# tachyon-beep/keisei

Hardware: AMD Instinct MI355X
Metric: PPO samples/sec, se_resnet 40x256 on 50x9x9 (higher is better)
Workload: dtype bf16; 1 GPU; se_resnet 40x256 KataGo-PPO minibatch step (gather+fwd+loss+bwd+clip+Adam), minibatch 4096/GPU from a 16384-sample device-resident epoch dataset, obs 50x9x9; per_gpu_batch=4096, global_batch=4096, parallelism=dp1

## Files before the change

keisei_amd/csrc/common.h:

```cpp
#pragma once
#include <hip/hip_runtime.h>
#include <stdint.h>

#define KA_OK 0
#define KA_ERR_ARG (-1)
#define KA_ERR_HIP (-2)
#define KA_ERR_UNSUPPORTED (-3)

#define KA_DTYPE_F32 0
#define KA_DTYPE_BF16 1

#define KA_BOARD 81
#define KA_PADBOARD 121

typedef __attribute__((ext_vector_type(8))) __bf16 bf16x8;
typedef __attribute__((ext_vector_type(4))) __bf16 bf16x4;
typedef __attribute__((ext_vector_type(4))) float f32x4;
typedef __attribute__((ext_vector_type(2))) float f32x2;

struct bf16_t { uint16_t v; };

void ka_set_error(const char* fmt, ...);
int ka_check_launch(const char* what);
#define KA_REQUIRE(cond, ...) do { if (!(cond)) { ka_set_error(__VA_ARGS__); return KA_ERR_ARG; } } while (0)

#include <atomic>
inline int ka_big_lds_once(const void* func, std::atomic<unsigned long long>& done, const char* what) {
    int dev = 0;
    if (hipGetDevice(&dev) != hipSuccess) { ka_set_error("%s: hipGetDevice failed", what); return KA_ERR_HIP; }
    const unsigned long long bit = 1ull << (dev & 63);
    if (done.load(std::memory_order_acquire) & bit) return KA_OK;
    if (hipFuncSetAttribute(func, hipFuncAttributeMaxDynamicSharedMemorySize, 160 * 1024) != hipSuccess) {
        ka_set_error("%s: hipFuncSetAttribute failed on device %d", what, dev);
        return KA_ERR_HIP;
    }
    done.fetch_or(bit, std::memory_order_release);
    return KA_OK;
}

#include <stdlib.h>
inline const char* ka_diag_env(const char* name) {
#ifdef KA_DIAG
    return getenv(name);
#else
    (void)name;
    return nullptr;
#endif
}

#define KA_OPTIONS(X)                                                                                                      \
    X(CONV_P) X(CONV_MT) X(CONV_PC2) X(CONV_PC2_SKIP) X(CONV_PC2_STAG) X(CONV_CORNER_IN) X(CONV_P_STAG) X(CONV_P_PRIO) X(CONV_P_WGS) X(CONV_P_NPW) X(CONV_WM) X(CONV_KC)       \
    X(CONV_NTW) X(CONV_STAGGER) X(CONV_PRIO) X(WGRAD_TN) X(WGRAD_WGS) X(WGRAD_STAG) X(WGRAD_LEAN) X(BOARD_PAIRS) X(TF_LDS_EPI) X(TF_K256) X(TF_BIG)    \
    X(TF_MAP2D) X(TF_ATTN_LDS) X(TF_ATTN_ONE) X(TAIL_FWD_KB) X(TAIL_GATE_P4)
enum KaOpt {
#define KA_OPT_ENUM(n) KA_OPT_##n,
    KA_OPTIONS(KA_OPT_ENUM)
#undef KA_OPT_ENUM
    KA_OPT_COUNT
};
struct KaOptVal { int set, val; };
const KaOptVal* ka_opts();
inline bool ka_opt_set(KaOpt o) { return ka_opts()[o].set != 0; }
inline int ka_opt(KaOpt o, int dflt) { const KaOptVal v = ka_opts()[o]; return v.set ? v.val : dflt; }

std::atomic<unsigned long long*>& ka_debug_stamps();

enum KaConvRoute {
    KA_RT_CONV,
    KA_RT_PC,
    KA_RT_PC2,
    KA_RT_PC2_CORNER_IN,
    KA_RT_PC2_CORNER_OUT,
    KA_RT_CORNER,
    KA_RT_WGRAD_LEAN,
    KA_RT_WGRAD_TILED,
    KA_RT_COUNT
};
void ka_conv_route(int r);

__device__ __forceinline__ float bf2f(uint16_t h) { return __uint_as_float(((uint32_t)h) << 16); }
__device__ __forceinline__ uint16_t f2bf(float f) {
    __bf16 b = (__bf16)f;
    return __builtin_bit_cast(uint16_t, b);
}

template <typename T> struct Elem;
template <> struct Elem<float> {
    static constexpr int kSize = 4;
    static constexpr int kPer16 = 4;
    static constexpr int kDtype = KA_DTYPE_F32;
    typedef f32x4 vec16;
    static __device__ __forceinline__ float ld(const float* p) { return *p; }
    static __device__ __forceinline__ void st(float* p, float v) { *p = v; }
    static __device__ __forceinline__ void unpack(const vec16& v, float* f) {
        f[0] = v[0]; f[1] = v[1]; f[2] = v[2]; f[3] = v[3];
    }
    static __device__ __forceinline__ vec16 pack(const float* f) { vec16 v = {f[0], f[1], f[2], f[3]}; return v; }
};
template <> struct Elem<bf16_t> {
    static constexpr int kSize = 2;
    static constexpr int kPer16 = 8;
    static constexpr int kDtype = KA_DTYPE_BF16;
    typedef bf16x8 vec16;
    static __device__ __forceinline__ float ld(const bf16_t* p) { return bf2f(p->v); }
    static __device__ __forceinline__ void st(bf16_t* p, float v) { p->v = f2bf(v); }
    static __device__ __forceinline__ void unpack(const vec16& v, float* f) {
#pragma unroll
        for (int i = 0; i < 8; ++i) f[i] = (float)v[i];
    }
    static __device__ __forceinline__ vec16 pack(const float* f) {
        vec16 v;
#pragma unroll
        for (int i = 0; i < 8; ++i) v[i] = (__bf16)f[i];
        return v;
    }
};

template <typename T> __device__ __forceinline__ f32x2 ld2(const T* p);
template <> __device__ __forceinline__ f32x2 ld2<float>(const float* p) { return *reinterpret_cast<const f32x2*>(p); }
template <> __device__ __forceinline__ f32x2 ld2<bf16_t>(const bf16_t* p) {
    uint32_t u = *reinterpret_cast<const uint32_t*>(p);
    f32x2 r = {__uint_as_float(u << 16), __uint_as_float(u & 0xffff0000u)};
    return r;
}
template <typename T> __device__ __forceinline__ void st2(T* p, f32x2 v);
template <> __device__ __forceinline__ void st2<float>(float* p, f32x2 v) { *reinterpret_cast<f32x2*>(p) = v; }
template <> __device__ __forceinline__ void st2<bf16_t>(bf16_t* p, f32x2 v) {
    uint32_t u = (uint32_t)f2bf(v[0]) | ((uint32_t)f2bf(v[1]) << 16);
// ... 85 lines not shown
```

keisei_amd/csrc/conv3x3.hip:

```cpp
#include <stdlib.h>
#include <utility>
#include "common.h"

static std::atomic<long long> g_conv_routes[KA_RT_COUNT];
void ka_conv_route(int r) { g_conv_routes[r].fetch_add(1, std::memory_order_relaxed); }

namespace {

constexpr int kNB = 2;
constexpr int kPW = 17;
constexpr int kBoardStride = 193;
constexpr int kLdsSquares = kBoardStride + 11 * kPW;
constexpr int kImgSquares1 = 10 * kPW + 11;
constexpr int kZeroSquares = 2 * (kPW + 1) + 1;
__device__ __forceinline__ int lds_square(int b, int p) { return b * kBoardStride + (p / 9 + 1) * kPW + (p % 9) + 1; }
constexpr int kMTW = 6;

__host__ __device__ __forceinline__ int chan_of(int nt, int s, int NT) {
    return ((nt | 1) < NT) ? (nt >> 1) * 32 + (s >> 2) * 8 + (nt & 1) * 4 + (s & 3) : nt * 16 + s;
}

__device__ __forceinline__ float row_sum16(float v) {
    v += __int_as_float(__builtin_amdgcn_update_dpp(0, __float_as_int(v), 0xB1, 0xF, 0xF, true));
    v += __int_as_float(__builtin_amdgcn_update_dpp(0, __float_as_int(v), 0x4E, 0xF, 0xF, true));
// ... 765 lines not shown
                        const float d = (in && y * esc[e] + esh[e] > 0.f) ? (float)db : 0.f;
                        t1[e] += d; t2[e] += d * ((y - emu[e]) * eis[e]);
                        o[e] = (__bf16)d;
                    }
                    if (j == 0) o0[mt] = o;
                    else if (in) {
                        bf16x8 o8;
#pragma unroll
                        for (int e = 0; e < 4; ++e) { o8[e] = o0[mt][e]; o8[4 + e] = o[e]; }
                        *reinterpret_cast<bf16x8*>(static_cast<char*>(a.out) + ((size_t)(bb * KA_BOARD + p) * a.Cout + cb0) * 2) = o8;
                    }
                }
#pragma unroll
                for (int e = 0; e < 4; ++e) { t1[e] = row_sum16(t1[e]); t2[e] = row_sum16(t2[e]); }
                if (rl == 0) {
                    *reinterpret_cast<f32x4*>(a.ep_s1 + (size_t)bb * a.Cout + cb0 + 4 * j) = f32x4{t1[0], t1[1], t1[2], t1[3]};
                    *reinterpret_cast<f32x4*>(a.ep_s2 + (size_t)bb * a.Cout + cb0 + 4 * j) = f32x4{t2[0], t2[1], t2[2], t2[3]};
                }
            }
            wfrag(0, 0, w0); wfrag(0, 1, w1); wfrag(0, 2, w2);
        }
    }
}

template <bool TWO, bool MASKED, int NPW, int MT, bool STAG = false>
static int launch_conv_pc_form(const ConvArgs& a, int grid, size_t lds, hipStream_t st, const char* what) {
    static std::atomic<unsigned long long> done{0};
    if (int rc = ka_big_lds_once(reinterpret_cast<const void*>(&conv3x3_pc_kernel<TWO, MASKED, NPW, MT, STAG>), done, what)) return rc;
    hipLaunchKernelGGL((conv3x3_pc_kernel<TWO, MASKED, NPW, MT, STAG>), dim3(grid), dim3(512 + 64 * NPW), lds, st, a);
    return ka_check_launch(what);
}
static int launch_conv_pc(ConvArgs a, hipStream_t st) {
    a.tune_stagger = 0; a.tune_prio = 0;
    if (const char* e = ka_diag_env("KA_CONV_P_ABL")) a.tune_stagger = atoi(e);
    a.tune_prio = ka_opt(KA_OPT_CONV_P_PRIO, 0);
    ka_conv_route(KA_RT_PC);
    int grid = 256;
    if (const int v = ka_opt(KA_OPT_CONV_P_WGS, 0); v > 0) grid = v;
    if (grid > a.B) grid = a.B;
    const int stag = ka_opt(KA_OPT_CONV_P_STAG, 0);
#define KA_PC_FORM(TWO_, MASKED_, NPW_, LDS_, WHAT_)                                                         \
    (a.mt5 ? ((stag && !MASKED_) ? launch_conv_pc_form<TWO_, false, NPW_, 5, true>(a, grid, LDS_, st, WHAT_ ", 5 row tiles, staggered") \
                                 : launch_conv_pc_form<TWO_, MASKED_, NPW_, 5>(a, grid, LDS_, st, WHAT_ ", 5 row tiles"))            \
           : launch_conv_pc_form<TWO_, MASKED_, NPW_, kMTW>(a, grid, LDS_, st, WHAT_))
    if (a.in2 && a.ep_y) return KA_PC_FORM(true, true, 4, kPcLdsMasked, "conv3x3 (pc, masked)");
    if (a.in2) return KA_PC_FORM(true, false, 4, kPcLds, "conv3x3 (pc, two-tensor)");
    if (ka_opt_set(KA_OPT_CONV_P_NPW) ? ka_opt(KA_OPT_CONV_P_NPW, 4) == 2 : (a.in_scale || a.relu || a.in_bias))
        return KA_PC_FORM(false, false, 2, kPcLds, "conv3x3 (pc, 2 staging waves)");
    return KA_PC_FORM(false, false, 4, kPcLds, "conv3x3 (pc)");
#undef KA_PC_FORM
}

typedef __attribute__((ext_vector_type(2))) unsigned u32x2;
template <int C, int MT>
__device__ __forceinline__ void conv_epilogue_masked_pair(const ConvArgs& a, f32x4 (&acc)[2 * MT][2], int b0, bool has_b1, int nt0, int r, int q) {
    constexpr int ROWB = C * 2, NT = C / 16;
    const int cb[2] = {chan_of(nt0, 4 * q, NT), chan_of(nt0 + 1, 4 * q, NT)};
    const char* yb = static_cast<const char*>(a.ep_y) + (size_t)b0 * (KA_BOARD * ROWB);
    char* ob = static_cast<char*>(a.out) + (size_t)b0 * (KA_BOARD * ROWB);
    const int lo[2] = {r * ROWB + cb[0] * 2, r * ROWB + cb[1] * 2};
    auto live = [&](int mt) { return MT == 5 || mt < 5 || r == 0; };
    u32x2 yA[MT], yB[MT];
    auto yload = [&](int b, int j, u32x2 (&y)[MT]) {
#pragma unroll
        for (int mt = 0; mt < MT; ++mt) y[mt] = live(mt) ? *reinterpret_cast<const u32x2*>(yb + b * (KA_BOARD * ROWB) + lo[j] + mt * 16 * ROWB) : u32x2{0u, 0u};
    };
    f32x4 cA[2], cB[2];
    yload(0, 0, yA);
    cA[0] = *reinterpret_cast<const f32x4*>(a.ep_scale + cb[0]); cA[1] = *reinterpret_cast<const f32x4*>(a.ep_shift + cb[0]);
    if (a.bsum) {
#pragma unroll
        for (int b = 0; b < 2; ++b)
#pragma unroll
            for (int j = 0; j < 2; ++j) {
                float s0[4] = {0.f, 0.f, 0.f, 0.f};
#pragma unroll
                for (int mt = 0; mt < MT; ++mt)
#pragma unroll
                    for (int i = 0; i < 4; ++i) s0[i] += live(mt) ? acc[MT * b + mt][j][i] : 0.f;
#pragma unroll
                for (int i = 0; i < 4; ++i) s0[i] = row_sum16(s0[i]);
                if (r == 0 && (b == 0 || has_b1)) *reinterpret_cast<f32x4*>(a.bsum + (b0 + b) * C + cb[j]) = f32x4{s0[0], s0[1], s0[2], s0[3]};
            }
    }
    yload(0, 1, yB);
    cB[0] = *reinterpret_cast<const f32x4*>(a.ep_scale + cb[1]); cB[1] = *reinterpret_cast<const f32x4*>(a.ep_shift + cb[1]);
    auto process = [&](int b, int j, const u32x2 (&y)[MT], const f32x4 (&c)[2]) {
        const f32x4 emu = *reinterpret_cast<const f32x4*>(a.ep_mean + cb[j]), eis = *reinterpret_cast<const f32x4*>(a.ep_invstd + cb[j]);
        float t1[4] = {0.f, 0.f, 0.f, 0.f}, t2[4] = {0.f, 0.f, 0.f, 0.f};
#pragma unroll
        for (int mt = 0; mt < MT; ++mt) {
            u32x2 o;
#pragma unroll
            for (int h = 0; h < 2; ++h) {
                const unsigned yw = y[mt][h];
                const float y0 = __uint_as_float(yw << 16), y1 = __uint_as_float(yw & 0xffff0000u);
                typedef __attribute__((ext_vector_type(2))) __bf16 bf16x2;
                const bf16x2 dbp = {(__bf16)acc[MT * b + mt][j][2 * h], (__bf16)acc[MT * b + mt][j][2 * h + 1]};
                const unsigned dw = __builtin_bit_cast(unsigned, dbp);
                const float d0 = (live(mt) && y0 * c[0][2 * h] + c[1][2 * h] > 0.f) ? __uint_as_float(dw << 16) : 0.f;
                const float d1 = (live(mt) && y1 * c[0][2 * h + 1] + c[1][2 * h + 1] > 0.f) ? __uint_as_float(dw & 0xffff0000u) : 0.f;
                t1[2 * h] += d0; t1[2 * h + 1] += d1;
                t2[2 * h] = fmaf(d0, y0, t2[2 * h]); t2[2 * h + 1] = fmaf(d1, y1, t2[2 * h + 1]);
                o[h] = (__float_as_uint(d0) >> 16) | __float_as_uint(d1);
            }
            if (live(mt)) *reinterpret_cast<u32x2*>(ob + b * (KA_BOARD * ROWB) + lo[j] + mt * 16 * ROWB) = o;
        }
#pragma unroll
        for (int e = 0; e < 4; ++e) {
            t1[e] = row_sum16(t1[e]);
            t2[e] = (row_sum16(t2[e]) - emu[e] * t1[e]) * eis[e];
        }
        if (r == 0) {
            *reinterpret_cast<f32x4*>(a.ep_s1 + (b0 + b) * C + cb[j]) = f32x4{t1[0], t1[1], t1[2], t1[3]};
            *reinterpret_cast<f32x4*>(a.ep_s2 + (b0 + b) * C + cb[j]) = f32x4{t2[0], t2[1], t2[2], t2[3]};
        }
    };
    process(0, 0, yA, cA);
    if (has_b1) yload(1, 0, yA);
    process(0, 1, yB, cB);
    if (has_b1) {
        yload(1, 1, yB);
        process(1, 0, yA, cA);
        process(1, 1, yB, cB);
    }
}

__device__ __forceinline__ void ld4x8_l2(const float* const (&p)[8], f32x4 (&v)[8]) {
    asm volatile("global_load_dwordx4 %0, %8, off sc1\n\t"
                 "global_load_dwordx4 %1, %9, off sc1\n\t"
                 "global_load_dwordx4 %2, %10, off sc1\n\t"
                 "global_load_dwordx4 %3, %11, off sc1\n\t"
                 "global_load_dwordx4 %4, %12, off sc1\n\t"
                 "global_load_dwordx4 %5, %13, off sc1\n\t"
                 "global_load_dwordx4 %6, %14, off sc1\n\t"
                 "global_load_dwordx4 %7, %15, off sc1\n\t"
                 "s_waitcnt vmcnt(0)"
                 : "=&v"(v[0]), "=&v"(v[1]), "=&v"(v[2]), "=&v"(v[3]), "=&v"(v[4]), "=&v"(v[5]), "=&v"(v[6]), "=&v"(v[7])
                 : "v"(p[0]), "v"(p[1]), "v"(p[2]), "v"(p[3]), "v"(p[4]), "v"(p[5]), "v"(p[6]), "v"(p[7])
                 : "memory");
}
__device__ __forceinline__ void corner_tile_epilogue(const ConvArgs& a, const f32x4 (&acc)[2], int bb, bool live, int nt0, int q) {
    if (!live) return;
    int cb[2];
    f32x4 pbs[2], psq[2], ps1[2], ps2[2];
    {
        const float* any = a.bsum ? a.bsum : reinterpret_cast<const float*>(a.wpack);
        const float* src[8];
#pragma unroll
        for (int j = 0; j < 2; ++j) {
            cb[j] = chan_of(nt0 + j, 4 * q, 16);
            const size_t srow = (size_t)bb * 256 + cb[j];
            src[j] = a.bsum ? a.bsum + srow : any;
            src[2 + j] = a.sqpart ? a.sqpart + srow : any;
            src[4 + j] = a.ep_y ? a.ep_s1 + srow : any;
            src[6 + j] = a.ep_y ? a.ep_s2 + srow : any;
        }
        f32x4 got[8];
        ld4x8_l2(src, got);
#pragma unroll
        for (int j = 0; j < 2; ++j) { pbs[j] = got[j]; psq[j] = got[2 + j]; ps1[j] = got[4 + j]; ps2[j] = got[6 + j]; }
    }
#pragma unroll
    for (int j = 0; j < 2; ++j) {
// ... 69 lines not shown
struct P2Seq { unsigned char s[216], t[216]; int n; };
constexpr P2Seq make_p2seq(bool skip, int ntiles) {
    P2Seq Q{};
    Q.n = 0;
    for (int s = 0; s < 18; ++s)
        for (int t = 0; t < ntiles; ++t)
            if (!(skip && p2_skip(t, s >> 1))) { Q.s[Q.n] = (unsigned char)s; Q.t[Q.n] = (unsigned char)t; ++Q.n; }
    return Q;
}

__device__ __forceinline__ void conv_epilogue_pair(const ConvArgs& a, f32x4 (&acc)[10][2], const unsigned (&sqp)[3], int b0, bool has_b1,
                                                   int nt0, int r, int q) {
    const int cb[2] = {chan_of(nt0, 4 * q, 16), chan_of(nt0 + 1, 4 * q, 16)};
    const bool isO = r >= 4 && r < 12;
    if (a.bsum || a.sqpart) {
#pragma unroll
        for (int j = 0; j < 2; ++j) {
#pragma unroll
            for (int b = 0; b < 2; ++b) {
                float s[4] = {0.f, 0.f, 0.f, 0.f}, ss[4] = {0.f, 0.f, 0.f, 0.f};
#pragma unroll
                for (int t = 0; t < 10; ++t) {
                    if (t >= 4 && (t >= 7) != (b == 1)) continue;
#pragma unroll
                    for (int i = 0; i < 4; ++i) {
                        float v = acc[t][j][i];
                        if (t < 4) v = (isO == (b == 1)) ? v : 0.f;
                        s[i] += v; ss[i] += v * v;
                    }
                }
#pragma unroll
                for (int i = 0; i < 4; ++i) { s[i] = row_sum16(s[i]); ss[i] = row_sum16(ss[i]); }
                if (r == 0 && (b == 0 || has_b1)) {
                    if (a.bsum) *reinterpret_cast<f32x4*>(a.bsum + (size_t)(b0 + b) * 256 + cb[j]) = f32x4{s[0], s[1], s[2], s[3]};
                    if (a.sqpart) *reinterpret_cast<f32x4*>(a.sqpart + (size_t)(b0 + b) * 256 + cb[j]) = f32x4{ss[0], ss[1], ss[2], ss[3]};
                }
                __builtin_amdgcn_sched_barrier(0);
            }
        }
    }
#pragma unroll
    for (int t = 0; t < 10; ++t) {
        const int bd = t < 4 ? (isO ? 1 : 0) : (t < 7 ? 0 : 1);
        if (bd && !has_b1) continue;
        bf16x8 o;
#pragma unroll
        for (int i = 0; i < 4; ++i) { o[i] = (__bf16)acc[t][0][i]; o[4 + i] = (__bf16)acc[t][1][i]; }
        const int sq = (int)((sqp[t >> 2] >> (8 * (t & 3))) & 0xffu);
        *reinterpret_cast<bf16x8*>(static_cast<char*>(a.out) + (size_t)b0 * (KA_BOARD * 512) + ((bd * KA_BOARD + sq) * 256 + cb[0]) * 2) = o;
        __builtin_amdgcn_sched_barrier(0);
    }
}

template <int C, int MT, bool TWO, bool MASKED, int NPW, bool SKIP = false, bool STAG = false, bool GATED = false>
__global__ __launch_bounds__((C / 32 + NPW) * 64) void conv3x3_pc2_kernel(ConvArgs a) {
    static_assert(!GATED || (TWO && MASKED && !SKIP && !STAG), "the gated input is conv2's data gradient: two-tensor, masked");
    static_assert(!(SKIP && MASKED), "the border-tile layout is built for the register-only epilogue");
    static_assert((C == 256 && MT == 5) || (C == 128 && MT == 6 && !SKIP), "shapes this kernel is built for");
    constexpr int NMW = C / 32, NCH = C / 64, NTILE = C / 16, KSG = C / 32, ROWB = C * 2, NTL = 2 * MT;
    constexpr int NT_ = (NMW + NPW) * 64, NP = 64 * NPW;
    constexpr int kHalf = KA_BOARD * 8, kPieces = 2 * kHalf;
    constexpr int KP = (kPieces + NP - 1) / NP;
    extern __shared__ __attribute__((aligned(16))) char smem[];
    const int tid = threadIdx.x, lane = tid & 63, wave = tid >> 6, r = lane & 15, q = lane >> 4;
    const int nwg = gridDim.x, npairs_all = (a.B + 1) >> 1;
    if ((int)blockIdx.x >= npairs_all) return;
    for (int i = tid; i < kP2Lds / 16; i += NT_) reinterpret_cast<uint4*>(smem)[i] = uint4{0, 0, 0, 0};
    const int npairs = (npairs_all - (int)blockIdx.x + nwg - 1) / nwg, nunits = NCH * npairs;
    if (!MASKED) a.ep_y = nullptr;
    __syncthreads();

    if (wave >= NMW) {
        const int pt = tid - NMW * 64, pc = pt & 7, swave = __builtin_amdgcn_readfirstlane(wave) - NMW;
        const bool has_aff = GATED || a.in_scale != nullptr;
        auto pair_rsrc = [&](const void* p, int b0, bool sized) {
            const unsigned nb = sized ? (unsigned)min(2, a.B - b0) * (KA_BOARD * ROWB) : 0u;
            return __builtin_amdgcn_make_buffer_rsrc(const_cast<char*>(static_cast<const char*>(p)) + (size_t)b0 * (KA_BOARD * ROWB), 0, nb,
                                                     0x00020000);
        };
        const int voff0 = (pt >> 3) * ROWB + pc * 16;
        int ldso[KP];
#pragma unroll
        for (int k = 0; k < KP; ++k) {
            const int row = min((pt + NP * k) >> 3, 2 * KA_BOARD - 1), j = row >= KA_BOARD ? 1 : 0;
            ldso[k] = j * kP2Img + lds_square(0, row - j * KA_BOARD) * kP2Stride + pc * 16;
        }
        auto live = [&](int k) { return (swave * 64 + NP * k) < kPieces; };
        const bool corner_in = C == 256 && MT == 5 && !MASKED && a.mt5 == 2;
        int cso[KP];
#pragma unroll
        for (int k = 0; k < KP; ++k) {
            const int row = min((pt + NP * k) >> 3, 2 * KA_BOARD - 1), j = row >= KA_BOARD ? 1 : 0, sq = row - j * KA_BOARD;
            const int ps = sq == 70 ? 0 : sq == 71 ? 1 : sq == 79 ? 2 : sq == 80 ? 3 : -1;
            cso[k] = (corner_in && ps >= 0 && pt + NP * k < kPieces) ? j * kP2SideRow + ps * 512 + pc * 16 : -1;
        }
        int chas = 0;
#pragma unroll
        for (int k = 0; k < KP; ++k) chas |= (__builtin_amdgcn_readfirstlane((int)(__ballot(cso[k] >= 0) != 0ull)) & 1) << k;
        bf16x8 pv[KP], pw[TWO ? KP : 1];
        auto stage_load = [&](int u) {
            const int b0 = __builtin_amdgcn_readfirstlane(2 * ((int)blockIdx.x + (u / NCH) * nwg)), c4 = u % NCH;
            const int soff = __builtin_amdgcn_readfirstlane(c4 * 128);
            const __amdgpu_buffer_rsrc_t r_in = pair_rsrc(a.in, b0, true), r_in2 = pair_rsrc(TWO ? a.in2 : a.in, b0, true);
#pragma unroll
            for (int k = 0; k < KP; ++k) {
                if (!live(k)) continue;
                const int vo = pt + NP * k < kPieces ? voff0 + k * (NP / 8) * ROWB : (int)0x7fffffff;
                pv[k] = __builtin_bit_cast(bf16x8, __builtin_amdgcn_raw_buffer_load_b128(r_in, vo, soff, 2));
                if (TWO) pw[TWO ? k : 0] = __builtin_bit_cast(bf16x8, __builtin_amdgcn_raw_buffer_load_b128(r_in2, vo, soff, 2));
            }
        };
        auto stage_write = [&](int u) __attribute__((always_inline)) {
            const int b0 = __builtin_amdgcn_readfirstlane(2 * ((int)blockIdx.x + (u / NCH) * nwg)), c4 = u % NCH, ch0 = c4 * 64 + pc * 8;
            const int soff = __builtin_amdgcn_readfirstlane(c4 * 128);
            const __amdgpu_buffer_rsrc_t r_out = pair_rsrc(a.in_out ? a.in_out : a.in, b0, a.in_out != nullptr);
            char* img = smem + (u & 1) * (2 * kP2Img);
            float sc[8], sh[8], k3[8], pb[2][8];
            {
                const f32x4 z = {0.f, 0.f, 0.f, 0.f}, o = {1.f, 1.f, 1.f, 1.f};
                const float* shp = GATED ? a.in_scale + C : a.in_shift;
                const float* k3p = GATED ? a.in_scale + 2 * C : a.in_k3;
                const f32x4 s0 = has_aff ? *reinterpret_cast<const f32x4*>(a.in_scale + ch0) : o, s1 = has_aff ? *reinterpret_cast<const f32x4*>(a.in_scale + ch0 + 4) : o;
                const f32x4 t0 = has_aff ? *reinterpret_cast<const f32x4*>(shp + ch0) : z, t1 = has_aff ? *reinterpret_cast<const f32x4*>(shp + ch0 + 4) : z;
                const f32x4 u0 = TWO ? *reinterpret_cast<const f32x4*>(k3p + ch0) : z, u1 = TWO ? *reinterpret_cast<const f32x4*>(k3p + ch0 + 4) : z;
                const bool bias = !TWO && a.in_bias;
                const f32x4 p00 = bias ? *reinterpret_cast<const f32x4*>(a.in_bias + (size_t)b0 * C + ch0) : z;
                const f32x4 p01 = bias ? *reinterpret_cast<const f32x4*>(a.in_bias + (size_t)b0 * C + ch0 + 4) : z;
                const bool b1 = bias && b0 + 1 < a.B;
                const f32x4 p10 = b1 ? *reinterpret_cast<const f32x4*>(a.in_bias + (size_t)(b0 + 1) * C + ch0) : z;
                const f32x4 p11 = b1 ? *reinterpret_cast<const f32x4*>(a.in_bias + (size_t)(b0 + 1) * C + ch0 + 4) : z;
#pragma unroll
                for (int e = 0; e < 4; ++e) {
                    sc[e] = s0[e]; sc[4 + e] = s1[e]; sh[e] = t0[e]; sh[4 + e] = t1[e]; k3[e] = u0[e]; k3[4 + e] = u1[e];
                    pb[0][e] = p00[e]; pb[0][4 + e] = p01[e]; pb[1][e] = p10[e]; pb[1][4 + e] = p11[e];
                }
            }
            float gsc0[8], gsh0[8], gsc1[8], gsh1[8];
            if constexpr (GATED) {
                const f32x4 z = {0.f, 0.f, 0.f, 0.f};
                const float* gp = a.in_bias + (size_t)b0 * C + ch0;
                const float* ap = gp + (size_t)a.B * C;
                const bool b1 = b0 + 1 < a.B;
                const f32x4 g00 = *reinterpret_cast<const f32x4*>(gp), g01 = *reinterpret_cast<const f32x4*>(gp + 4);
                const f32x4 a00 = *reinterpret_cast<const f32x4*>(ap), a01 = *reinterpret_cast<const f32x4*>(ap + 4);
                const f32x4 g10 = b1 ? *reinterpret_cast<const f32x4*>(gp + C) : z, g11 = b1 ? *reinterpret_cast<const f32x4*>(gp + C + 4) : z;
                const f32x4 a10 = b1 ? *reinterpret_cast<const f32x4*>(ap + C) : z, a11 = b1 ? *reinterpret_cast<const f32x4*>(ap + C + 4) : z;
#pragma unroll
                for (int e = 0; e < 4; ++e) {
                    gsc0[e] = g00[e] * sc[e]; gsc0[4 + e] = g01[e] * sc[4 + e];
                    gsh0[e] = fmaf(a00[e], sc[e], sh[e]); gsh0[4 + e] = fmaf(a01[e], sc[4 + e], sh[4 + e]);
                    gsc1[e] = g10[e] * sc[e]; gsc1[4 + e] = g11[e] * sc[4 + e];
                    gsh1[e] = fmaf(a10[e], sc[e], sh[e]); gsh1[4 + e] = fmaf(a11[e], sc[4 + e], sh[4 + e]);
                }
            }
#pragma unroll
            for (int k = 0; k < KP; ++k) {
                if (!live(k)) continue;
                const int i = pt + NP * k;
                if (i >= kPieces) continue;
                const int j = i >= kHalf ? 1 : 0;
                bf16x8 v = pv[k];
                if (TWO) {
                    const bool jlo = NP * (k + 1) <= kHalf, jhi = NP * k >= kHalf;
#pragma unroll
                    for (int e = 0; e < 8; ++e) {
                        float se_ = sc[e], he_ = sh[e];
                        if constexpr (GATED) {
                            const float c0 = gsc0[e], c1 = gsc1[e], h0 = gsh0[e], h1 = gsh1[e];
                            se_ = jlo ? c0 : jhi ? c1 : (j ? c1 : c0);
                            he_ = jlo ? h0 : jhi ? h1 : (j ? h1 : h0);
                        }
                        v[e] = (__bf16)fmaf((float)pw[TWO ? k : 0][e], k3[e], fmaf((float)v[e], se_, he_));
                    }
                    if (b0 + j >= a.B) v = bf16x8{};
                    __builtin_amdgcn_raw_buffer_store_b128(__builtin_bit_cast(__attribute__((ext_vector_type(4))) unsigned, v), r_out,
                                                           voff0 + k * (NP / 8) * ROWB, soff, 0);
                } else if (has_aff || a.relu || a.in_bias) {
#pragma unroll
                    for (int e = 0; e < 8; e += 2) {
                        f32x2 f = {(float)v[e], (float)v[e + 1]};
                        if (has_aff) f = __builtin_elementwise_fma(f, f32x2{sc[e], sc[e + 1]}, f32x2{sh[e], sh[e + 1]});
                        if (a.relu) f = __builtin_elementwise_max(f, f32x2{0.f, 0.f});
                        if (a.in_bias) f += j ? f32x2{pb[1][e], pb[1][e + 1]} : f32x2{pb[0][e], pb[0][e + 1]};
                        v[e] = (__bf16)f[0]; v[e + 1] = (__bf16)f[1];
                    }
                    if (b0 + j >= a.B) v = bf16x8{};
                    if constexpr (C == 256) __builtin_amdgcn_raw_buffer_store_b128(__builtin_bit_cast(__attribute__((ext_vector_type(4))) unsigned, v), r_out,
                                                           voff0 + k * (NP / 8) * ROWB, soff, 0);
                }
                *reinterpret_cast<bf16x8*>(img + ldso[k]) = v;
            }
        };
        auto side_write = [&](int u) {
            if constexpr (C == 256 && MT == 5) {
                if (!corner_in) return;
                const char* img = smem + (u & 1) * (2 * kP2Img);
                const int side0 = kP2Side + 2 * ((u / NCH) % kP2SideSlots) * kP2SideRow + (u % NCH) * 128;
#pragma unroll
                for (int k = 0; k < KP; ++k) {
                    if (!live(k) || !((chas >> k) & 1)) continue;
                    const bf16x8 t = *reinterpret_cast<const bf16x8*>(img + ldso[k]);
                    *reinterpret_cast<bf16x8*>(smem + (cso[k] >= 0 ? side0 + cso[k] : kP2Dump)) = t;
                }
            }
        };
        auto stage = [&](int u) __attribute__((always_inline)) { stage_load(u); stage_write(u); side_write(u); };
        stage(0);
        KA_LDS_BARRIER();
        if constexpr (STAG) {
            for (int v = 1; v < nunits; ++v) {
                stage_load(v);
                KA_LDS_BARRIER();
                stage_write(v);
                side_write(v);
                KA_LDS_BARRIER();
            }
            KA_LDS_BARRIER();
            KA_LDS_BARRIER();
            return;
        }
        for (int u = 0; u < nunits; ++u) {
            if (u + 1 < nunits) stage(u + 1);
            KA_LDS_BARRIER();
        }
        return;
    }

    const __amdgpu_buffer_rsrc_t wrsrc = __builtin_amdgcn_make_buffer_rsrc(const_cast<void*>(a.wpack), 0, 9 * KSG * NTILE * 1024, 0x00020000);
    const int wlane = __builtin_amdgcn_readfirstlane(wave) * 2048 + lane * 16;
    auto wfrag = [&](int c4, int s, bf16x8 (&f)[2]) {
        if (s >= 18) { s -= 18; c4 = (c4 + 1) % NCH; }
        const int tap = s >> 1, ks = c4 * 2 + (s & 1);
        const int so = __builtin_amdgcn_readfirstlane(((tap * KSG + ks) * NTILE) * 1024);
        f[0] = __builtin_bit_cast(bf16x8, __builtin_amdgcn_raw_buffer_load_b128(wrsrc, wlane, so, 0));
        f[1] = __builtin_bit_cast(bf16x8, __builtin_amdgcn_raw_buffer_load_b128(wrsrc, wlane + 1024, so, 0));
    };
    constexpr int NRB = SKIP ? 10 : MT;
    int rowbase[NRB];
    unsigned sqp[3] = {0u, 0u, 0u};
#pragma unroll
    for (int t = 0; t < NRB; ++t) {
        if (SKIP) {
            const int sq = kP2Perm.sq[t][r];
            sqp[t >> 2] |= (unsigned)sq << (8 * (t & 3));
            const int bd = t < 4 ? ((r >= 4 && r < 12) ? 1 : 0) : (t < 7 ? 0 : 1);
            rowbase[t] = bd * kP2Img + lds_square(0, sq) * kP2Stride + q * 16 - kP2Base;
        } else {
            const int p = t * 16 + r;
            rowbase[t] = (p < KA_BOARD ? lds_square(0, p) : kPW + 13) * kP2Stride + q * 16 - kP2Base;
        }
    }
    auto frag_off = [&](int t) { return SKIP ? rowbase[SKIP ? t : 0] : rowbase[t % MT] + (t / MT) * kP2Img; };
    bf16x8 wr[3][2];
    wfrag(0, 0, wr[0]); wfrag(0, 1, wr[1]);
    f32x4 acc[NTL][2];
    KA_LDS_BARRIER();
    if (a.stamps && tid == 0) {
        a.stamps[blockIdx.x * 8 + 0] = __builtin_amdgcn_s_memtime();
        a.stamps[blockIdx.x * 8 + 3] = __builtin_amdgcn_s_memrealtime();
    }
    const bool late = STAG && __builtin_amdgcn_readfirstlane(wave) >= NMW / 2;
    if (late) KA_LDS_BARRIER();
    for (int u = 0; u < nunits; ++u) {
        const int c4 = u % NCH;
        if (!c4) {
#pragma unroll
            for (int t = 0; t < NTL; ++t) { acc[t][0] = f32x4{0.f, 0.f, 0.f, 0.f}; acc[t][1] = f32x4{0.f, 0.f, 0.f, 0.f}; }
        }
        const char* img = smem;
        constexpr P2Seq Q = make_p2seq(SKIP, NTL);
        constexpr int R = MASKED ? 5 : 8;
        bf16x8 fa[R];
        auto frag_at = [&](auto n_) {
            constexpr int n = decltype(n_)::value, s = Q.s[n], t = Q.t[n], tap = s >> 1;
            constexpr int toff = kP2Base + ((tap / 3 - 1) * kPW + (tap % 3 - 1)) * kP2Stride + (s & 1) * 64;
            fa[n % R] = *reinterpret_cast<const bf16x8*>(img + frag_off(t) + toff);
        };
        static_for<R>(frag_at);
        static_for<Q.n>([&](auto n_) {
            constexpr int n = decltype(n_)::value, s = Q.s[n], t = Q.t[n];
            if constexpr (n == 0 || Q.s[n > 0 ? n - 1 : 0] != s) {
                __builtin_amdgcn_sched_barrier(0);
                if constexpr (STAG && s == 9) KA_LDS_BARRIER();
                if (!(MASKED && c4 == NCH - 1 && s >= 16)) wfrag(c4, s + 2, wr[(s + 2) % 3]);
                __builtin_amdgcn_sched_barrier(0);
            }
            acc[t][0] = __builtin_amdgcn_mfma_f32_16x16x32_bf16(wr[s % 3][0], fa[n % R], acc[t][0], 0, 0, 0);
            acc[t][1] = __builtin_amdgcn_mfma_f32_16x16x32_bf16(wr[s % 3][1], fa[n % R], acc[t][1], 0, 0, 0);
            __builtin_amdgcn_sched_group_barrier(0x008, 2, 0);
            if constexpr (n + R < Q.n) {
                frag_at(std::integral_constant<int, n + R>{});
                __builtin_amdgcn_sched_group_barrier(0x100, 1, 0);
            }
        });
        __builtin_amdgcn_sched_barrier(0);
        if (c4 == NCH - 1) {
            const int b0 = 2 * ((int)blockIdx.x + (u / NCH) * nwg);
            if constexpr (MASKED) {
                int rl = r, ql = q;
                asm volatile("" : "+v"(rl), "+v"(ql));
                conv_epilogue_masked_pair<C, MT>(a, acc, b0, b0 + 1 < a.B, wave * 2, rl, ql);
                wfrag(0, 0, wr[0]); wfrag(0, 1, wr[1]);
            } else if constexpr (SKIP) {
                if constexpr (SKIP) conv_epilogue_pair(a, acc, sqp, b0, b0 + 1 < a.B, wave * 2, r, q);
            } else {
                conv_epilogue<bf16_t, 2, MT>(a, reinterpret_cast<f32x4 (&)[MT][2]>(acc[0]), b0, wave * 2, NTILE, r, q);
                if (b0 + 1 < a.B) conv_epilogue<bf16_t, 2, MT>(a, reinterpret_cast<f32x4 (&)[MT][2]>(acc[MT]), b0 + 1, wave * 2, NTILE, r, q);
            }
            if constexpr (C == 256 && MT == 5 && !SKIP && !STAG && !MASKED) {
                const int pidx = u / NCH;
                if (a.mt5 == 2 && ((pidx & 7) == 7 || pidx == npairs - 1)) {
                    const int g0 = pidx & ~7;
                    const int pr = g0 + (r >> 1), prc = min(pr, pidx);
                    const char* arow = smem + kP2Side + (2 * (prc % kP2SideSlots) + (r & 1)) * kP2SideRow + q * 16;
                    auto cw = [&](int step, bf16x8 (&f)[2]) {
                        const int ps = (step >> 2) & 3, tap = ps < 2 ? ps : ps + 1, ks = (step >> 4) * 4 + (step & 3);
                        const int so = __builtin_amdgcn_readfirstlane(((tap * KSG + ks) * NTILE) * 1024);
                        f[0] = __builtin_bit_cast(bf16x8, __builtin_amdgcn_raw_buffer_load_b128(wrsrc, wlane, so, 0));
                        f[1] = __builtin_bit_cast(bf16x8, __builtin_amdgcn_raw_buffer_load_b128(wrsrc, wlane + 1024, so, 0));
                    };
                    constexpr int kAh = 8;
                    bf16x8 wq[kAh][2];
#pragma unroll
                    for (int s2 = 0; s2 < kAh; ++s2) cw(s2, wq[s2]);
                    f32x4 cacc[2] = {f32x4{0.f, 0.f, 0.f, 0.f}, f32x4{0.f, 0.f, 0.f, 0.f}};
#pragma unroll
                    for (int step = 0; step < 32; ++step) {
                        const bf16x8 w0 = wq[step % kAh][0], w1 = wq[step % kAh][1];
                        if (step + kAh < 32) cw(step + kAh, wq[step % kAh]);
                        const int ps = (step >> 2) & 3, ks = (step >> 4) * 4 + (step & 3);
                        const bf16x8 af = *reinterpret_cast<const bf16x8*>(arow + ps * 512 + ks * 64);
                        cacc[0] = __builtin_amdgcn_mfma_f32_16x16x32_bf16(w0, af, cacc[0], 0, 0, 0);
                        cacc[1] = __builtin_amdgcn_mfma_f32_16x16x32_bf16(w1, af, cacc[1], 0, 0, 0);
                    }
                    const int bb = 2 * ((int)blockIdx.x + pr * nwg) + (r & 1);
                    asm volatile("s_waitcnt vmcnt(0)" ::: "memory");
                    corner_tile_epilogue(a, cacc, bb, pr <= pidx && bb < a.B, wave * 2, q);
                }
            }
        }
#pragma unroll
        for (int t = 0; t < NRB; ++t) rowbase[t] += (u & 1) ? -2 * kP2Img : 2 * kP2Img;
        if (!(late && u == nunits - 1)) KA_LDS_BARRIER();
    }
    if (a.stamps && tid == 0) {
        a.stamps[blockIdx.x * 8 + 7] = __builtin_amdgcn_s_memtime();
        a.stamps[blockIdx.x * 8 + 4] = __builtin_amdgcn_s_memrealtime();
    }
}

template <int C, int MT, bool TWO, bool MASKED, int NPW, bool SKIP = false, bool STAG = false, bool GATED = false>
static int launch_conv_pc2_form(const ConvArgs& a, hipStream_t st, const char* what) {
    static std::atomic<unsigned long long> done{0};
    if (int rc = ka_big_lds_once(reinterpret_cast<const void*>(&conv3x3_pc2_kernel<C, MT, TWO, MASKED, NPW, SKIP, STAG, GATED>), done, what)) return rc;
    const int pairs = (a.B + 1) / 2, grid = pairs < 256 ? pairs : 256;
    hipLaunchKernelGGL((conv3x3_pc2_kernel<C, MT, TWO, MASKED, NPW, SKIP, STAG, GATED>), dim3(grid), dim3((C / 32 + NPW) * 64),
                       C == 256 ? kP2LdsCorner : kP2Lds, st, a);
    return ka_check_launch(what);
}
static int launch_conv_pc2(const ConvArgs& a, hipStream_t st) {
    ka_conv_route(a.Cin == 128 ? KA_RT_PC2 : (a.mt5 == 2 ? KA_RT_PC2_CORNER_IN : KA_RT_PC2_CORNER_OUT));
    if (a.in2 && a.in_bias) {
        KA_REQUIRE(a.in2 && a.ep_y, "conv3x3: the gated input comes with the two-tensor transform and the masked epilogue");
        if (a.Cin == 128) return launch_conv_pc2_form<128, 6, true, true, 4, false, false, true>(a, st, "conv3x3 (two boards per unit, 128 channels, gated two-tensor, masked)");
        return launch_conv_pc2_form<256, 5, true, true, 4, false, false, true>(a, st, "conv3x3 (two boards per unit, gated two-tensor, masked)");
    }
    if (a.Cin == 128) {
        if (a.in2 && a.ep_y) return launch_conv_pc2_form<128, 6, true, true, 4>(a, st, "conv3x3 (two boards per unit, 128 channels, two-tensor, masked)");
        if (a.in2) return launch_conv_pc2_form<128, 6, true, false, 4>(a, st, "conv3x3 (two boards per unit, 128 channels, two-tensor)");
        return launch_conv_pc2_form<128, 6, false, false, 4>(a, st, "conv3x3 (two boards per unit, 128 channels)");
    }
    const bool skip = ka_opt(KA_OPT_CONV_PC2_SKIP, 0) != 0;
    const bool stag = ka_opt(KA_OPT_CONV_PC2_STAG, 0) != 0;
    if (stag && !skip) {
        if (a.in2 && a.ep_y) return launch_conv_pc2_form<256, 5, true, true, 4, false, true>(a, st, "conv3x3 (two boards per unit, two-tensor, masked, staggered)");
        if (a.in2) return launch_conv_pc2_form<256, 5, true, false, 4, false, true>(a, st, "conv3x3 (two boards per unit, two-tensor, staggered)");
        return launch_conv_pc2_form<256, 5, false, false, 4, false, true>(a, st, "conv3x3 (two boards per unit, staggered)");
    }
    if (a.in2 && a.ep_y) return launch_conv_pc2_form<256, 5, true, true, 4>(a, st, "conv3x3 (two boards per unit, two-tensor, masked)");
    if (a.in2) return skip ? launch_conv_pc2_form<256, 5, true, false, 4, true>(a, st, "conv3x3 (two boards per unit, two-tensor, border tiles)")
                           : launch_conv_pc2_form<256, 5, true, false, 4>(a, st, "conv3x3 (two boards per unit, two-tensor)");
    return skip ? launch_conv_pc2_form<256, 5, false, false, 4, true>(a, st, "conv3x3 (two boards per unit, border tiles)")
                : launch_conv_pc2_form<256, 5, false, false, 4>(a, st, "conv3x3 (two boards per unit)");
}

constexpr int kCornerBoards = 32, kCornerStride = 4 * 512 + 16;
constexpr int kCornerLds = kCornerBoards * kCornerStride;

__global__ __launch_bounds__(512) void conv3x3_corner_kernel(ConvArgs a) {
    extern __shared__ __attribute__((aligned(16))) char cs[];
    const int tid = threadIdx.x, lane = tid & 63, wave = tid >> 6, r = lane & 15, q = lane >> 4;
    const int b0 = blockIdx.x * kCornerBoards;
    const int rt = wave & 1, nt0 = blockIdx.y * 8 + (wave >> 1) * 2;
    const char* wl = static_cast<const char*>(a.wpack) + (size_t)nt0 * 1024 + lane * 16;
    auto wfrag = [&](int step, int j) {
        const int kc = step >> 4, ps = (step >> 2) & 3, ks = kc * 4 + (step & 3), tap = ps < 2 ? ps : ps + 1;
        return *reinterpret_cast<const bf16x8*>(wl + (size_t)((tap * 8 + ks) * 16 + j) * 1024);
    };
    constexpr int kAhead = 12;
    bf16x8 wq[kAhead][2];
#pragma unroll
    for (int s2 = 0; s2 < kAhead; ++s2) { wq[s2][0] = wfrag(s2, 0); wq[s2][1] = wfrag(s2, 1); }
    const bool has_aff = a.in_scale != nullptr;
    const int pc = tid & 31, ch0 = pc * 8;
    {
        bf16x8 pv[8], pw[8];
#pragma unroll
        for (int k = 0; k < 8; ++k) {
            const int i = tid + 512 * k, bl = i >> 7, ps = (i >> 5) & 3, bb = min(b0 + bl, a.B - 1);
            const int p = ps == 0 ? 70 : ps == 1 ? 71 : ps == 2 ? 79 : 80;
            const size_t off = (((size_t)bb * KA_BOARD + p) * 256 + ch0) * 2;
            pv[k] = *reinterpret_cast<const bf16x8*>(static_cast<const char*>(a.in) + off);
            pw[k] = a.in2 ? *reinterpret_cast<const bf16x8*>(static_cast<const char*>(a.in2) + off) : bf16x8{};
        }
        float sc[8], sh[8], k3[8];
#pragma unroll
        for (int e = 0; e < 8; ++e) { sc[e] = 1.f; sh[e] = 0.f; k3[e] = 0.f; }
// ... 296 lines not shown
```

Measured before the change: 44010 samples/s.

## Route gated masked conv epilogue through LDS to producer waves

Adds an ELDS variant of the 256-channel gated masked pc2 conv kernel, now the default. The MFMA waves write bf16 accumulators into a new LDS staging buffer and compute only the batch-norm sums. The producer waves then run the masked ReLU-gradient epilogue, reading y and the coefficients from LDS and writing coalesced 16-byte stores. This offloads epilogue work from the compute waves and frees registers for more fragment prefetch (R=8), at the cost of more LDS, extra barriers and more producer work.

```diff
diff --git a/keisei_amd/csrc/common.h b/keisei_amd/csrc/common.h
--- a/keisei_amd/csrc/common.h
+++ b/keisei_amd/csrc/common.h
@@ -49,7 +49,7 @@
 }
 
 #define KA_OPTIONS(X)                                                                                                      \
-    X(CONV_P) X(CONV_MT) X(CONV_PC2) X(CONV_PC2_SKIP) X(CONV_PC2_STAG) X(CONV_CORNER_IN) X(CONV_P_STAG) X(CONV_P_PRIO) X(CONV_P_WGS) X(CONV_P_NPW) X(CONV_WM) X(CONV_KC)       \
+    X(CONV_P) X(CONV_MT) X(CONV_PC2) X(CONV_PC2_SKIP) X(CONV_PC2_STAG) X(CONV_MASKED_LDS) X(CONV_CORNER_IN) X(CONV_P_STAG) X(CONV_P_PRIO) X(CONV_P_WGS) X(CONV_P_NPW) X(CONV_WM) X(CONV_KC)       \
     X(CONV_NTW) X(CONV_STAGGER) X(CONV_PRIO) X(WGRAD_TN) X(WGRAD_WGS) X(WGRAD_STAG) X(WGRAD_LEAN) X(BOARD_PAIRS) X(TF_LDS_EPI) X(TF_K256) X(TF_BIG)    \
     X(TF_MAP2D) X(TF_ATTN_LDS) X(TF_ATTN_ONE) X(TAIL_FWD_KB) X(TAIL_GATE_P4)
 enum KaOpt {
@@ -74,6 +74,7 @@
     KA_RT_CORNER,
     KA_RT_WGRAD_LEAN,
     KA_RT_WGRAD_TILED,
+    KA_RT_PC2_MASKED_LDS,
     KA_RT_COUNT
 };
 void ka_conv_route(int r);
diff --git a/keisei_amd/csrc/conv3x3.hip b/keisei_amd/csrc/conv3x3.hip
--- a/keisei_amd/csrc/conv3x3.hip
+++ b/keisei_amd/csrc/conv3x3.hip
@@ -841,6 +841,18 @@
 }
 
 typedef __attribute__((ext_vector_type(2))) unsigned u32x2;
+typedef __attribute__((ext_vector_type(4))) unsigned u32x4;
+template <typename L>
+__device__ __forceinline__ unsigned masked_word(float y0, float y1, unsigned dw, L live, float sc0, float sh0, float sc1, float sh1,
+                                                float& s1a, float& s1b, float& s2a, float& s2b) {
+    const float d0 = (live() && y0 * sc0 + sh0 > 0.f) ? __uint_as_float(dw << 16) : 0.f;
+    const float d1 = (live() && y1 * sc1 + sh1 > 0.f) ? __uint_as_float(dw & 0xffff0000u) : 0.f;
+    s1a += d0; s1b += d1;
+    s2a = fmaf(d0, y0, s2a); s2b = fmaf(d1, y1, s2b);
+    return (__float_as_uint(d0) >> 16) | __float_as_uint(d1);
+}
+__device__ __forceinline__ float masked_s2(float dy, float mean, float s1, float invstd) { return (dy - mean * s1) * invstd; }
+
 template <int C, int MT>
 __device__ __forceinline__ void conv_epilogue_masked_pair(const ConvArgs& a, f32x4 (&acc)[2 * MT][2], int b0, bool has_b1, int nt0, int r, int q) {
     constexpr int ROWB = C * 2, NT = C / 16;
@@ -886,19 +898,15 @@
                 const float y0 = __uint_as_float(yw << 16), y1 = __uint_as_float(yw & 0xffff0000u);
                 typedef __attribute__((ext_vector_type(2))) __bf16 bf16x2;
                 const bf16x2 dbp = {(__bf16)acc[MT * b + mt][j][2 * h], (__bf16)acc[MT * b + mt][j][2 * h + 1]};
-                const unsigned dw = __builtin_bit_cast(unsigned, dbp);
-                const float d0 = (live(mt) && y0 * c[0][2 * h] + c[1][2 * h] > 0.f) ? __uint_as_float(dw << 16) : 0.f;
-                const float d1 = (live(mt) && y1 * c[0][2 * h + 1] + c[1][2 * h + 1] > 0.f) ? __uint_as_float(dw & 0xffff0000u) : 0.f;
-                t1[2 * h] += d0; t1[2 * h + 1] += d1;
-                t2[2 * h] = fmaf(d0, y0, t2[2 * h]); t2[2 * h + 1] = fmaf(d1, y1, t2[2 * h + 1]);
-                o[h] = (__float_as_uint(d0) >> 16) | __float_as_uint(d1);
+                o[h] = masked_word(y0, y1, __builtin_bit_cast(unsigned, dbp), [&] { return live(mt); }, c[0][2 * h], c[1][2 * h], c[0][2 * h + 1], c[1][2 * h + 1],
+                                   t1[2 * h], t1[2 * h + 1], t2[2 * h], t2[2 * h + 1]);
             }
             if (live(mt)) *reinterpret_cast<u32x2*>(ob + b * (KA_BOARD * ROWB) + lo[j] + mt * 16 * ROWB) = o;
         }
 #pragma unroll
         for (int e = 0; e < 4; ++e) {
             t1[e] = row_sum16(t1[e]);
-            t2[e] = (row_sum16(t2[e]) - emu[e] * t1[e]) * eis[e];
+            t2[e] = masked_s2(row_sum16(t2[e]), emu[e], t1[e], eis[e]);
         }
         if (r == 0) {
             *reinterpret_cast<f32x4*>(a.ep_s1 + (b0 + b) * C + cb[j]) = f32x4{t1[0], t1[1], t1[2], t1[3]};
@@ -1074,9 +1082,86 @@
     }
 }
 
-template <int C, int MT, bool TWO, bool MASKED, int NPW, bool SKIP = false, bool STAG = false, bool GATED = false>
+constexpr int kP2EStride = 256 * 2 + 16;
+constexpr int kP2ERows = 80;
+constexpr int kP2E = kP2Lds, kP2ECoef = kP2E + kP2ERows * kP2EStride, kP2LdsE = kP2ECoef + 4 * 256 * 4;
+static_assert(kP2LdsE <= 160 * 1024, "the epilogue buffer fits behind the images");
+struct MaskedPass { u32x4 y[5]; };
+__device__ __forceinline__ void conv_masked_pass_request(const ConvArgs& a, int bb, int r, int col, MaskedPass& P) {
+    const char* yb = static_cast<const char*>(a.ep_y) + (size_t)bb * (KA_BOARD * 512);
+    const unsigned lo = (unsigned)(r * 512 + col * 16);
+#pragma unroll
+    for (int mt = 0; mt < 5; ++mt) P.y[mt] = *reinterpret_cast<const u32x4*>(yb + (lo + mt * 16 * 512));
+}
+__device__ __forceinline__ void conv_masked_pass(const ConvArgs& a, const char* E, const float* coef, int bb, int r, int col, const MaskedPass& P) {
+    const f32x4 sc[2] = {*reinterpret_cast<const f32x4*>(coef + col * 8), *reinterpret_cast<const f32x4*>(coef + col * 8 + 4)};
+    const f32x4 sh[2] = {*reinterpret_cast<const f32x4*>(coef + 256 + col * 8), *reinterpret_cast<const f32x4*>(coef + 256 + col * 8 + 4)};
+    const char* Er = E + r * kP2EStride + col * 16;
+    u32x4 e = *reinterpret_cast<const u32x4*>(Er);
+    float t1[8] = {0.f, 0.f, 0.f, 0.f, 0.f, 0.f, 0.f, 0.f}, t2[8] = {0.f, 0.f, 0.f, 0.f, 0.f, 0.f, 0.f, 0.f};
+    char* ob = static_cast<char*>(a.out) + (size_t)bb * (KA_BOARD * 512);
+    const unsigned lo = (unsigned)(r * 512 + col * 16);
+#pragma unroll
+    for (int mt = 0; mt < 5; ++mt) {
+        const u32x4 ec = e;
+        if (mt < 4) e = *reinterpret_cast<const u32x4*>(Er + (mt + 1) * 16 * kP2EStride);
+        u32x4 o;
+#pragma unroll
+        for (int h = 0; h < 4; ++h) {
+            const unsigned yw = P.y[mt][h];
+            const float y0 = __uint_as_float(yw << 16), y1 = __uint_as_float(yw & 0xffff0000u);
+            const int j = h >> 1, i = 2 * (h & 1);
+            o[h] = masked_word(y0, y1, ec[h], [] { return true; }, sc[j][i], sh[j][i], sc[j][i + 1], sh[j][i + 1],
+                               t1[2 * h], t1[2 * h + 1], t2[2 * h], t2[2 * h + 1]);
+        }
+        *reinterpret_cast<u32x4*>(ob + (lo + mt * 16 * 512)) = o;
+        __builtin_amdgcn_sched_barrier(0);
+    }
+    const f32x4 mu[2] = {*reinterpret_cast<const f32x4*>(coef + 512 + col * 8), *reinterpret_cast<const f32x4*>(coef + 512 + col * 8 + 4)};
+    const f32x4 is[2] = {*reinterpret_cast<const f32x4*>(coef + 768 + col * 8), *reinterpret_cast<const f32x4*>(coef + 768 + col * 8 + 4)};
+#pragma unroll
+    for (int c = 0; c < 8; ++c) {
+        t1[c] = row_sum16(t1[c]);
+        t2[c] = masked_s2(row_sum16(t2[c]), mu[c >> 2][c & 3], t1[c], is[c >> 2][c & 3]);
+    }
+    if (r == 0) {
+        float* s1 = a.ep_s1 + (size_t)bb * 256 + col * 8;
+        float* s2 = a.ep_s2 + (size_t)bb * 256 + col * 8;
+        *reinterpret_cast<f32x4*>(s1) = f32x4{t1[0], t1[1], t1[2], t1[3]}; *reinterpret_cast<f32x4*>(s1 + 4) = f32x4{t1[4], t1[5], t1[6], t1[7]};
+        *reinterpret_cast<f32x4*>(s2) = f32x4{t2[0], t2[1], t2[2], t2[3]}; *reinterpret_cast<f32x4*>(s2 + 4) = f32x4{t2[4], t2[5], t2[6], t2[7]};
+    }
+}
+__device__ __forceinline__ void conv_masked_bsum_pair(const ConvArgs& a, f32x4 (&acc)[10][2], int b0, bool has_b1, int nt0, int r, int q) {
+    if (!a.bsum) return;
+    const int cb[2] = {chan_of(nt0, 4 * q, 16), chan_of(nt0 + 1, 4 * q, 16)};
+#pragma unroll
+    for (int b = 0; b < 2; ++b)
+#pragma unroll
+        for (int j = 0; j < 2; ++j) {
+            float s0[4] = {0.f, 0.f, 0.f, 0.f};
+#pragma unroll
+            for (int mt = 0; mt < 5; ++mt)
+#pragma unroll
+                for (int i = 0; i < 4; ++i) s0[i] += acc[5 * b + mt][j][i];
+#pragma unroll
+            for (int i = 0; i < 4; ++i) s0[i] = row_sum16(s0[i]);
+            if (r == 0 && (b == 0 || has_b1)) *reinterpret_cast<f32x4*>(a.bsum + (b0 + b) * 256 + cb[j]) = f32x4{s0[0], s0[1], s0[2], s0[3]};
+        }
+}
+__device__ __forceinline__ void conv_masked_lay(char* E, const f32x4 (&acc)[10][2], int b, int wave, int r, int q) {
+#pragma unroll
+    for (int mt = 0; mt < 5; ++mt) {
+        bf16x8 o;
+#pragma unroll
+        for (int i = 0; i < 4; ++i) { o[i] = (__bf16)acc[5 * b + mt][0][i]; o[4 + i] = (__bf16)acc[5 * b + mt][1][i]; }
+        *reinterpret_cast<bf16x8*>(E + (mt * 16 + r) * kP2EStride + wave * 64 + q * 16) = o;
+    }
+}
+
+template <int C, int MT, bool TWO, bool MASKED, int NPW, bool SKIP = false, bool STAG = false, bool GATED = false, bool ELDS = false>
 __global__ __launch_bounds__((C / 32 + NPW) * 64) void conv3x3_pc2_kernel(ConvArgs a) {
     static_assert(!GATED || (TWO && MASKED && !SKIP && !STAG), "the gated input is conv2's data gradient: two-tensor, masked");
+    static_assert(!ELDS || (GATED && C == 256 && MT == 5 && NPW == 4), "the epilogue through LDS is built for the 256-channel gated masked form");
     static_assert(!(SKIP && MASKED), "the border-tile layout is built for the register-only epilogue");
     static_assert((C == 256 && MT == 5) || (C == 128 && MT == 6 && !SKIP), "shapes this kernel is built for");
     constexpr int NMW = C / 32, NCH = C / 64, NTILE = C / 16, KSG = C / 32, ROWB = C * 2, NTL = 2 * MT;
@@ -1090,6 +1175,12 @@
     for (int i = tid; i < kP2Lds / 16; i += NT_) reinterpret_cast<uint4*>(smem)[i] = uint4{0, 0, 0, 0};
     const int npairs = (npairs_all - (int)blockIdx.x + nwg - 1) / nwg, nunits = NCH * npairs;
     if (!MASKED) a.ep_y = nullptr;
+    if constexpr (ELDS) {
+        float* coef = reinterpret_cast<float*>(smem + kP2ECoef);
+        for (int i = tid; i < 256; i += NT_) {
+            coef[i] = a.ep_scale[i]; coef[256 + i] = a.ep_shift[i]; coef[512 + i] = a.ep_mean[i]; coef[768 + i] = a.ep_invstd[i];
+        }
+    }
     __syncthreads();
 
     if (wave >= NMW) {
@@ -1124,10 +1215,12 @@
             const int b0 = __builtin_amdgcn_readfirstlane(2 * ((int)blockIdx.x + (u / NCH) * nwg)), c4 = u % NCH;
             const int soff = __builtin_amdgcn_readfirstlane(c4 * 128);
             const __amdgpu_buffer_rsrc_t r_in = pair_rsrc(a.in, b0, true), r_in2 = pair_rsrc(TWO ? a.in2 : a.in, b0, true);
+            int vb = voff0;
+            if constexpr (ELDS) asm volatile("" : "+v"(vb));
 #pragma unroll
             for (int k = 0; k < KP; ++k) {
                 if (!live(k)) continue;
-                const int vo = pt + NP * k < kPieces ? voff0 + k * (NP / 8) * ROWB : (int)0x7fffffff;
+                const int vo = pt + NP * k < kPieces ? vb + k * (NP / 8) * ROWB : (int)0x7fffffff;
                 pv[k] = __builtin_bit_cast(bf16x8, __builtin_amdgcn_raw_buffer_load_b128(r_in, vo, soff, 2));
                 if (TWO) pw[TWO ? k : 0] = __builtin_bit_cast(bf16x8, __builtin_amdgcn_raw_buffer_load_b128(r_in2, vo, soff, 2));
             }
@@ -1137,6 +1230,8 @@
             const int soff = __builtin_amdgcn_readfirstlane(c4 * 128);
             const __amdgpu_buffer_rsrc_t r_out = pair_rsrc(a.in_out ? a.in_out : a.in, b0, a.in_out != nullptr);
             char* img = smem + (u & 1) * (2 * kP2Img);
+            int vb = voff0;
+            if constexpr (ELDS) asm volatile("" : "+v"(vb));
             float sc[8], sh[8], k3[8], pb[2][8];
             {
                 const f32x4 z = {0.f, 0.f, 0.f, 0.f}, o = {1.f, 1.f, 1.f, 1.f};
@@ -1196,7 +1291,7 @@
                     }
                     if (b0 + j >= a.B) v = bf16x8{};
                     __builtin_amdgcn_raw_buffer_store_b128(__builtin_bit_cast(__attribute__((ext_vector_type(4))) unsigned, v), r_out,
-                                                           voff0 + k * (NP / 8) * ROWB, soff, 0);
+                                                           vb + k * (NP / 8) * ROWB, soff, 0);
                 } else if (has_aff || a.relu || a.in_bias) {
 #pragma unroll
                     for (int e = 0; e < 8; e += 2) {
@@ -1243,6 +1338,25 @@
         }
         for (int u = 0; u < nunits; ++u) {
             if (u + 1 < nunits) stage(u + 1);
+            if constexpr (ELDS) {
+                if (u % NCH == NCH - 1) {
+                    const int b0 = __builtin_amdgcn_readfirstlane(2 * ((int)blockIdx.x + (u / NCH) * nwg));
+                    const bool has_b1 = b0 + 1 < a.B;
+                    int er = lane & 15, ecol = swave * 8 + (lane >> 4);
+                    asm volatile("" : "+v"(er), "+v"(ecol));
+                    const float* coef = reinterpret_cast<const float*>(smem + kP2ECoef);
+                    MaskedPass P[2];
+                    conv_masked_pass_request(a, b0, er, ecol, P[0]);
+                    conv_masked_pass_request(a, b0, er, ecol + 4, P[1]);
+                    KA_LDS_BARRIER();
+                    conv_masked_pass(a, smem + kP2E, coef, b0, er, ecol, P[0]);
+                    conv_masked_pass(a, smem + kP2E, coef, b0, er, ecol + 4, P[1]);
+                    if (has_b1) { conv_masked_pass_request(a, b0 + 1, er, ecol, P[0]); conv_masked_pass_request(a, b0 + 1, er, ecol + 4, P[1]); }
+                    KA_LDS_BARRIER();
+                    KA_LDS_BARRIER();
+                    if (has_b1) { conv_masked_pass(a, smem + kP2E, coef, b0 + 1, er, ecol, P[0]); conv_masked_pass(a, smem + kP2E, coef, b0 + 1, er, ecol + 4, P[1]); }
+                }
+            }
             KA_LDS_BARRIER();
         }
         return;
@@ -1291,7 +1405,7 @@
         }
         const char* img = smem;
         constexpr P2Seq Q = make_p2seq(SKIP, NTL);
-        constexpr int R = MASKED ? 5 : 8;
+        constexpr int R = (MASKED && !ELDS) ? 5 : 8;
         bf16x8 fa[R];
         auto frag_at = [&](auto n_) {
             constexpr int n = decltype(n_)::value, s = Q.s[n], t = Q.t[n], tap = s >> 1;
@@ -1304,7 +1418,7 @@
             if constexpr (n == 0 || Q.s[n > 0 ? n - 1 : 0] != s) {
                 __builtin_amdgcn_sched_barrier(0);
                 if constexpr (STAG && s == 9) KA_LDS_BARRIER();
-                if (!(MASKED && c4 == NCH - 1 && s >= 16)) wfrag(c4, s + 2, wr[(s + 2) % 3]);
+                if (!(MASKED && !ELDS && c4 == NCH - 1 && s >= 16)) wfrag(c4, s + 2, wr[(s + 2) % 3]);
                 __builtin_amdgcn_sched_barrier(0);
             }
             acc[t][0] = __builtin_amdgcn_mfma_f32_16x16x32_bf16(wr[s % 3][0], fa[n % R], acc[t][0], 0, 0, 0);
@@ -1318,7 +1432,19 @@
         __builtin_amdgcn_sched_barrier(0);
         if (c4 == NCH - 1) {
             const int b0 = 2 * ((int)blockIdx.x + (u / NCH) * nwg);
-            if constexpr (MASKED) {
+            if constexpr (ELDS) {
+                int rl = r, ql = q;
+                asm volatile("" : "+v"(rl), "+v"(ql));
+                const bool has_b1 = b0 + 1 < a.B;
+                const int wv = __builtin_amdgcn_readfirstlane(wave);
+                char* E = smem + kP2E;
+                conv_masked_bsum_pair(a, acc, b0, has_b1, wv * 2, rl, ql);
+                conv_masked_lay(E, acc, 0, wv, rl, ql);
+                KA_LDS_BARRIER();
+                KA_LDS_BARRIER();
+                if (has_b1) conv_masked_lay(E, acc, 1, wv, rl, ql);
+                KA_LDS_BARRIER();
+            } else if constexpr (MASKED) {
                 int rl = r, ql = q;
                 asm volatile("" : "+v"(rl), "+v"(ql));
                 conv_epilogue_masked_pair<C, MT>(a, acc, b0, b0 + 1 < a.B, wave * 2, rl, ql);
@@ -1371,13 +1497,13 @@
     }
 }
 
-template <int C, int MT, bool TWO, bool MASKED, int NPW, bool SKIP = false, bool STAG = false, bool GATED = false>
+template <int C, int MT, bool TWO, bool MASKED, int NPW, bool SKIP = false, bool STAG = false, bool GATED = false, bool ELDS = false>
 static int launch_conv_pc2_form(const ConvArgs& a, hipStream_t st, const char* what) {
     static std::atomic<unsigned long long> done{0};
-    if (int rc = ka_big_lds_once(reinterpret_cast<const void*>(&conv3x3_pc2_kernel<C, MT, TWO, MASKED, NPW, SKIP, STAG, GATED>), done, what)) return rc;
+    if (int rc = ka_big_lds_once(reinterpret_cast<const void*>(&conv3x3_pc2_kernel<C, MT, TWO, MASKED, NPW, SKIP, STAG, GATED, ELDS>), done, what)) return rc;
     const int pairs = (a.B + 1) / 2, grid = pairs < 256 ? pairs : 256;
-    hipLaunchKernelGGL((conv3x3_pc2_kernel<C, MT, TWO, MASKED, NPW, SKIP, STAG, GATED>), dim3(grid), dim3((C / 32 + NPW) * 64),
-                       C == 256 ? kP2LdsCorner : kP2Lds, st, a);
+    hipLaunchKernelGGL((conv3x3_pc2_kernel<C, MT, TWO, MASKED, NPW, SKIP, STAG, GATED, ELDS>), dim3(grid), dim3((C / 32 + NPW) * 64),
+                       ELDS ? kP2LdsE : C == 256 ? kP2LdsCorner : kP2Lds, st, a);
     return ka_check_launch(what);
 }
 static int launch_conv_pc2(const ConvArgs& a, hipStream_t st) {
@@ -1385,6 +1511,10 @@
     if (a.in2 && a.in_bias) {
         KA_REQUIRE(a.in2 && a.ep_y, "conv3x3: the gated input comes with the two-tensor transform and the masked epilogue");
         if (a.Cin == 128) return launch_conv_pc2_form<128, 6, true, true, 4, false, false, true>(a, st, "conv3x3 (two boards per unit, 128 channels, gated two-tensor, masked)");
+        if (ka_opt(KA_OPT_CONV_MASKED_LDS, 1) != 0) {
+            ka_conv_route(KA_RT_PC2_MASKED_LDS);
+            return launch_conv_pc2_form<256, 5, true, true, 4, false, false, true, true>(a, st, "conv3x3 (two boards per unit, gated two-tensor, masked through LDS)");
+        }
         return launch_conv_pc2_form<256, 5, true, true, 4, false, false, true>(a, st, "conv3x3 (two boards per unit, gated two-tensor, masked)");
     }
     if (a.Cin == 128) {
```

New measurement: 44260 samples/s, median of 6. About the same (+0.6%).
